# hanruihua/RDA-planner

Hardware: AMD Instinct MI355X
Metric: MPC steps/sec (ADMM early stop or iter_num cap: see residuals), T=20, N_obs=200 (higher is better)
Workload: dtype f64; 1 GPU; north-star: acker rectangle robot, T=20, N_obs=200 static seeded polygons, E=4, iter_num=4, iter_threshold=0.2, ro1=200; parallelism=single GPU

## Files before the change

include/rda_hip.h:

```cpp
#ifndef RDA_HIP_H
#define RDA_HIP_H
#include <stdint.h>
#ifdef __cplusplus
extern "C" {
#endif

#define RDA_EMAX 8
#define RDA_RMAX 8
#define RDA_TMAX 64

typedef struct rda_cfg {
    int32_t T;
    int32_t N;
    int32_t E;
    int32_t R;
    int32_t dynamics;
    int32_t accelerated;
    int32_t iter_num;
    int32_t robot_norm2;
    double dt, L;
    double max_speed[2];
    double acce_bound[2];
    double iter_threshold;
    double ws, wu;
// ... 214 lines not shown
                                     double *states_log , double *u_log , int32_t *index_log ,
                                     rda_info *info_log , int32_t *arrived_at ,
                                     int32_t *nbox_log , double *clearance_log ,
                                     double *peer_clearance_log , int see, double gate, int window);
int  rda_fleet_track_boxes(rda_fleet *f, const int32_t *n , const double *boxes , int cap, double gate, int window,
                           double *vel_out );
int  rda_fleet_box_tracks(rda_fleet *f, int cap, int32_t *n , double *centres, double *vel, int32_t *age);
int  rda_fleet_reset_tracks(rda_fleet *f, const int32_t *which , int count);
int  rda_set_scan_split(rda_handle *h, double tol);
int  rda_fleet_set_scan_split(rda_fleet *f, double tol);
int  rda_debug_fleet_world(rda_fleet *f, double *geom, int32_t *n_total, int32_t *we);
int  rda_fleet_enqueue_range(rda_fleet *f, int k0, int k1);
int  rda_fleet_sync(rda_fleet *f);

int  rda_get_state(rda_handle *h, double *lam, double *mu, double *z, double *xi, double *zeta,
                   double *dis, double *a_lam, double *b_lam);
int  rda_set_state(rda_handle *h, const double *lam, const double *mu, const double *z,
                   const double *xi, const double *zeta, const double *dis,
                   const double *a_lam, const double *b_lam);
#define RDA_SU_HISTORY_INTS 8
int  rda_get_su_history(rda_handle *h, int32_t *hist , double *lam_keep );
int  rda_set_su_history(rda_handle *h, const int32_t *hist , const double *lam_keep );
int  rda_get_su_history_n(rda_handle *h, int32_t *hist, int n_hist, double *lam_keep );
int  rda_set_su_history_n(rda_handle *h, const int32_t *hist, int n_hist, const double *lam_keep );
int  rda_lmz_history_doubles(rda_handle *h);
int  rda_get_lmz_history(rda_handle *h, double *points, int32_t *valid);
int  rda_set_lmz_history(rda_handle *h, const double *points, const int32_t *valid);
int  rda_debug_su_prof(rda_handle *h, long long *out16);
int  rda_debug_su_trace(rda_handle *h, long long *out, int cap, int *n_out);
int  rda_debug_su_land(rda_handle *h, int32_t *out4);
int  rda_debug_su_land_n(rda_handle *h, int32_t *out, int n);
int  rda_debug_flush_supports(rda_handle *h);
int  rda_debug_slot_src(rda_handle *h, int32_t *src , int32_t *used);
int  rda_debug_worklist(rda_handle *h, int *rows);
int  rda_debug_alloc_fail(int n);
int  rda_debug_alloc_stats(long long *live_allocs, long long *live_bytes);

int  rda_shard_config(rda_handle *h, int rank, int world);
int  rda_shard_chunk_doubles(rda_handle *h);
int  rda_shard_get_chunk(rda_handle *h, double *host_chunk);
int  rda_shard_set_chunks(rda_handle *h, const double *host_all);
int  rda_shard_unique_id(rda_handle *h, void *out128);
int  rda_shard_comm_init(rda_handle *h, const void *uid128);
int  rda_shard_comm_count(rda_handle *h);
int  rda_admm_begin(rda_handle *h, const double *nom_s, const double *nom_u, const double *ref_s, double ref_speed);
int  rda_admm_su(rda_handle *h, int it, int *stopped);
int  rda_admm_lammuz(rda_handle *h);
int  rda_admm_finish(rda_handle *h, double *out_u, double *out_s, rda_info *info);

int  rda_lammuz_batch(int B, int E, int R, const double *A, const double *b, const int32_t *cone,
                      const double *p, const double *phi, const double *G, const double *h,
                      const double *xi, const double *zeta, const double *dbar, double ro2, double delta,
                      int accelerated, double *lam, double *mu, double *z, double *cmh);

int  rda_su_solve(const rda_cfg *cfg, const double *nom_s, const double *nom_u, const double *ref_s,
                  double ref_speed, const double *a, const double *cc, const double *g,
                  const double *d0, double *s, double *u, double *d, int32_t *ipm_iters);
int  rda_su_solve_opts(const rda_cfg *cfg, const rda_opts *opts, const double *nom_s, const double *nom_u, const double *ref_s,
                       double ref_speed, const double *a, const double *cc, const double *g,
                       const double *d0, double *s, double *u, double *d, int32_t *ipm_iters);

#ifdef __cplusplus
}
#endif
#endif
```

rda_planner_amd/_capi.py:

```python
import ctypes as C
import numpy as np

c_double_p = C.POINTER(C.c_double)
c_int_p = C.POINTER(C.c_int)


class Cfg(C.Structure):
    _fields_ = [("T", C.c_int), ("N", C.c_int), ("E", C.c_int), ("R", C.c_int),
                ("dynamics", C.c_int), ("accelerated", C.c_int), ("iter_num", C.c_int),
                ("robot_norm2", C.c_int),
                ("dt", C.c_double), ("L", C.c_double),
                ("max_speed", C.c_double * 2), ("acce_bound", C.c_double * 2),
                ("iter_threshold", C.c_double), ("ws", C.c_double), ("wu", C.c_double),
                ("slack_gain", C.c_double), ("max_sd", C.c_double), ("min_sd", C.c_double),
                ("ro1", C.c_double), ("ro2", C.c_double),
                ("delta", C.c_double), ("eps_u", C.c_double)]


class Opts(C.Structure):
    _fields_ = [("lmz_mode", C.c_int), ("tie_centre", C.c_int), ("lmz_mu", C.c_double), ("su_tol", C.c_double * 3), ("su_tol_early", C.c_double * 3), ("su_hard_warm", C.c_double * 2),
                ("lmz_warm", C.c_int), ("lmz_rows", C.c_int), ("lmz_dense_from", C.c_int), ("lmz_split", C.c_int),
                ("lmz_ip_rows", C.c_int), ("lmz_ip_warm", C.c_int), ("su_pre", C.c_int), ("su_light", C.c_int),
                ("su_warm_first", C.c_int), ("su_warm_cap", C.c_int), ("su_easy_max", C.c_int), ("su_easy_nopred", C.c_int),
                ("su_cold_from", C.c_int), ("su_cold_probe", C.c_int), ("zero_copy", C.c_int), ("early_finish", C.c_int),
# ... 77 lines not shown
    "fleet_rollout_peers_plan": "i hiDDIdiiDDDDINIDDDI",
    "fleet_rollout_last_plan":  "i hD",
    "fleet_peer_clearance": "i hDD",
    "fleet_upload_worlds":  "i hIiIIDD",
    "fleet_raycast":        "i hIDDDDDD",
    "fleet_rollout_lidar":  "i hiDDIdiiDIDDDDdiIiDDINIID",
    "fleet_raycast_peers":  "i hIDDDDDD",
    "fleet_rollout_lidar_peers": "i hiDDIdiiDIDDDDdiIiDDINIIDD",
    "fleet_upload_scans_tracked": "i hIDDDDDdiIIdi",
    "fleet_rollout_lidar_tracked": "i hiDDIdiiDIDDDDdiIiDDINIIDDidi",
    "fleet_track_boxes":    "i hIDidiD",
    "fleet_box_tracks":     "i hiIDDI",
    "fleet_reset_tracks":   "i hIi",
    "set_scan_split":       "i hd",
    "fleet_set_scan_split": "i hd",
    "debug_fleet_world":    "i hDII",
    "fleet_enqueue_range":  "i hii",
    "fleet_sync":           "i h",
    "get_state":            "i hDDDDDDDD",
    "set_state":            "i hDDDDDDDD",
    "get_su_history":       "i hID",
    "set_su_history":       "i hID",
    "get_su_history_n":     "i hIiD",
    "set_su_history_n":     "i hIiD",
    "lmz_history_doubles":  "i h",
    "get_lmz_history":      "i hDI",
    "set_lmz_history":      "i hDI",
    "debug_su_prof":        "i hQ",
    "debug_su_trace":       "i hQiI",
    "debug_su_land":        "i hI",
    "debug_su_land_n":      "i hIi",
    "debug_flush_supports": "i h",
    "debug_slot_src":       "i hII",
    "debug_worklist":       "i hI",
    "debug_alloc_fail":     "i i",
    "debug_alloc_stats":    "i QQ",
    "shard_config":         "i hii",
    "shard_chunk_doubles":  "i h",
    "shard_get_chunk":      "i hD",
    "shard_set_chunks":     "i hD",
    "shard_unique_id":      "i hh",
    "shard_comm_init":      "i hh",
    "shard_comm_count":     "i h",
    "admm_begin":           "i hDDDd",
    "admm_su":              "i hiI",
    "admm_lammuz":          "i h",
    "admm_finish":          "i hDDN",
    "lammuz_batch":         "i iiiDDIDDDDDDDddiDDDD",
    "su_solve":             "i CDDDdDDDDDDDI",
    "su_solve_opts":        "i CODDDdDDDDDDDI",
    "debug_lmz_clk":        "i hhi",
    "debug_lmz_stats":      "i hh",
}
PROFILING_ONLY = frozenset(("debug_lmz_clk", "debug_lmz_stats"))


def signature(proto, codes=CODES):
    ret, _, params = proto.partition(" ")
    return codes[ret], [codes[c] for c in params]


def declare(lib, prefix, table, codes=CODES):
    for name, proto in table.items():
        fn = getattr(lib, f"{prefix}_{name}", None)
        if fn is not None:
            fn.restype, fn.argtypes = signature(proto, codes)
# ... 87 lines not shown
```

rda_planner_amd/csrc/rda_hip.hip:

```cpp
#include <hip/hip_runtime.h>
#include <cfloat>
#include <climits>
#include <cstdio>
#include <cstdlib>
#include <cstring>
#include <vector>
#include <chrono>
#include <memory>
#include <dlfcn.h>
#include "../../include/rda_hip.h"
#include "host_buf.h"
#include "lammuz_device.h"
#include "lammuz_cp_device.h"
#include "lammuz_ip_device.h"
#include "su_device.h"
#include "scene_device.h"
#include "lidar_device.h"
#include "track_device.h"
#include "rollout_device.h"

#define HIPCHK(x) do { hipError_t e_ = (x); if (e_ != hipSuccess) { \
    fprintf(stderr, "librda_hip: %s failed: %s (%s:%d)\n", #x, hipGetErrorString(e_), __FILE__, __LINE__); return RDA_ERR_HIP; } } while (0)

struct Ctrl {
// ... 263 lines not shown
    if (blind_opportunity && cl.blind_ok >= 0) a.land_blind = 1;
    if (!hard && a.warm_mu0 > 0 && d.su_cold_from > 0 && cl.su_last > d.su_cold_from && cl.su_last < 99 && cl.su_probe % d.su_cold_probe != d.su_cold_probe - 1) a.warm_mu0 = 0;
#ifdef SU_TRACE
    a.t_entry = t_entry_; t_mark_[3] = clock64();
    for (int k = 0; k < 4; ++k) a.t_mark[k] = t_mark_[k];
#endif
    su::solve<TT>(a, smem_su, pre, true, res, ref_wait);
    if (tid == 0) {
        const int su_last = res.status == 0 ? res.iters : 99;
        d.ctrl->iters = it + 1;
        if (res.status != 0) d.ctrl->su_status = cl.su_status | (1 << it);
        d.ctrl->ipm_iters = cl.ipm_iters + res.iters;
        d.ctrl->su_last = su_last;
        d.ctrl->su_hardlike = res.rd0 > su::HARD_RD0;
        d.ctrl->su_probe = (d.su_cold_from > 0 && su_last > d.su_cold_from && su_last < 99) ? cl.su_probe + 1 : 0;
        d.ctrl->pose_ok = 0;
        if (a.land) {
            const bool easy1 = res.status == 0 && res.iters == 0 && res.rounds_all == 1;
            d.ctrl->land_easy = easy1 ? (cl.land_easy < 8 ? cl.land_easy + 1 : 8) : 0;
            if (res.land_rho > 0) d.ctrl->land_rho_prev = res.land_rho;
            if (blind_opportunity) d.ctrl->blind_ok = res.blind == 1 ? (cl.blind_ok < 4 ? cl.blind_ok + 1 : 4) : (res.blind == 2 ? -6 : (cl.blind_ok < 0 ? cl.blind_ok + 1 : cl.blind_ok));
        }
        if (a.land && res.status == 0) {
            int lh = cl.land_hard;
            if (res.land_rounds >= 3) lh = 4; else if (lh > 0) lh -= 1;
            d.ctrl->land_hard = lh;
        }
        if (lf_eligible && d.su_land_first == 2) {
            int cr = cl.spec_credit;
            if (res.spec == 1) cr = cr + 3 > 6 ? 6 : cr + 3; else if (res.spec == 2) cr -= 2; else if (cr < 0) cr += 1;
            d.ctrl->spec_credit = cr;
        }
    }
}

template <int TT> __global__ __launch_bounds__(su::NT) void k_su(Dev d, int it, const double *in_s, const double *in_u, Fin fin)
{
    warm_kernargs<sizeof(Dev) + 2 * sizeof(void *) + sizeof(int) + sizeof(Fin)>();
    su_body<TT>(d, it, in_s, in_u, d.ref, d.ref_speed, nullptr, 0, &fin);
}

__device__ __forceinline__ void finish_body(const Dev &d, const Fin &f)
{
    if (d.ctrl->finished) return;
    if (!d.ctrl->stop && d.ctrl->resi_iter != d.ctrl->iters) { ResPre none; double rd, rp; reduce_residuals(d, threadIdx.x, d.ctrl->iters, none, false, nullptr, rd, rp); }
    __syncthreads();
    publish_result(d, f);
}

__global__ __launch_bounds__(su::NT) void k_finish(Dev d, Fin f) { finish_body(d, f); }

__device__ __forceinline__ void begin_body(const Dev &d)
{
    if (threadIdx.x == 0) {
        d.ctrl->stop = 0; d.ctrl->iters = 0; d.ctrl->su_status = 0; d.ctrl->ipm_iters = 0; d.ctrl->lmz_fail = 0;
        d.ctrl->resi_dual = 0; d.ctrl->resi_pri = 0; d.ctrl->finished = 0; d.ctrl->wl_count = 0; d.ctrl->wlc_count = 0; d.ctrl->resi_iter = 0;
    }
}

__global__ void k_begin(Dev d) { begin_body(d); }

__device__ __forceinline__ void prepare_body(const Dev &d, lmz::WaveLDS *wl)
{
    const int lane = threadIdx.x & 63, wv = threadIdx.x >> 6, E = d.c.E;
    const int w = blockIdx.x * 4 + wv;
    if (w >= d.c.N * d.nt) return;
// ... 196 lines not shown
constexpr int LMZ_CLK_WORDS = 32;
__device__ int *g_lmz_faillog = nullptr;
#endif
template <int MODE = 0, bool CW = false> __device__ __forceinline__ void lammuz_body_rows(const Dev &d, const int block, const int nblocks, const int it, const Fin &fin)
{
#pragma clang fp contract(on)
    constexpr int WPB = GS / 4;
    constexpr bool LANES = CW;
    __shared__ lmz::WaveLDS wl[GS];
    __shared__ lmz::RobotLDS rb;
    __shared__ double rowv[MODE == 0 ? GS : 1][6];
    const int T = d.c.T, E = d.c.E, R = d.c.R;
#ifdef RDA_LMZ_CLK
    long long clk_prev = clock64(); const long long clk_in = clk_prev; bool clk_enum = false; const unsigned long long clk_wall_in = (unsigned long long)wall_clock64();
    unsigned long long *const clk_slot = g_lmz_clk ? g_lmz_clk + LMZ_CLK_WORDS * (size_t)(block * (GS / 4) + (threadIdx.x >> 6)) : nullptr;
    long long clk_sub = clk_prev;
#define LMZ_CLK(k) do { if (MODE == 0) { const long long now_ = clock64(); if (clk_slot && (threadIdx.x & 63) == 0) clk_slot[k] += (unsigned long long)(now_ - clk_prev); clk_prev = now_; clk_sub = now_; } } while (0)
#define LMZ_SUB(k) do { if (MODE == 0) { const long long now_ = clock64(); if (clk_slot && (threadIdx.x & 63) == 0) clk_slot[16 + (k)] += (unsigned long long)(now_ - clk_sub); clk_sub = now_; } } while (0)
#else
#define LMZ_CLK(k) do { } while (0)
#define LMZ_SUB(k) do { } while (0)
#endif
    int tb = 0, jb = 0;
    if (MODE != 2) { block_of(d, block, tb, jb); if (tb < 0) return; }
    const int lane = threadIdx.x & 63, wv = threadIdx.x >> 6, row = lane >> 4, gl = lane & 15;
    struct Early { double px, py, cs, sn, xi0, xi1, zeta, dbar, prev, vtx[4], A, b, G, h, zold, rv; int cone, src, hpar, hint, npv, nlv; unsigned char lamc[3], muc; } ey;
    if (MODE == 0) {
        const int nl0 = jb * GS + wv * 4 + row, nl = nl0 < d.Nlive ? nl0 : 0, n = d.rank * d.Nloc + nl;
        ey.src = (d.slot_src && n < d.src_used) ? d.slot_src[n] : -1;
        ey.hpar = d.ctrl->hint_par & 1;
        static_assert(64 * WPB >= 56, "one element of the robot tables per thread");
        if (LANES) { ey.muc = d.muc[(int)threadIdx.x < 40 ? threadIdx.x : 0]; ey.rv = (&d.rv[0][0])[(int)threadIdx.x < 56 ? threadIdx.x : 0]; }
    }
    if (LANES) {
        int stop = d.ctrl->stop;
        asm volatile("" : "+v"(ey.hpar), "+v"(stop));
        ey.hpar = __builtin_amdgcn_readfirstlane(ey.hpar);
        if (__builtin_amdgcn_readfirstlane(stop)) return;
    } else
    if (d.ctrl->stop) return;
    if (MODE == 2 && block * WPB >= d.ctrl->wl_count + (d.ctrl->wlc_count + 3) / 4) return;
    LMZ_CLK(0);
    if (MODE == 0) {
        const int t = tb, nl0 = jb * GS + wv * 4 + row, nl = nl0 < d.Nlive ? nl0 : 0, n = d.rank * d.Nloc + nl;
        const double *ps = d.pose + 4 * t;
        const size_t o = drow(d, n, t + 1), zi = drow(d, n, t), oc = (size_t)n * d.nt + (d.nt > 1 ? t + 1 : 0);
        ey.px = ps[0]; ey.py = ps[1]; ey.cs = ps[2]; ey.sn = ps[3];
        ey.xi0 = d.xi[2 * o]; ey.xi1 = d.xi[2 * o + 1]; ey.zeta = d.zeta[zi]; ey.dbar = d.dis[t]; ey.cone = d.cone[n];
        ey.zold = d.z[zi];
        ey.prev = *(gl < E ? &d.lam[o * E + gl] : (gl < E + R ? &d.mu[o * R + gl - E] : &d.lam[o * E]));
        {
            const size_t ao = ((size_t)n * d.nt + (d.nt > 1 ? t + 1 : 0)) * E;
            ey.A = d.A[ao * 2 + (gl < 2 * E ? gl : 0)]; ey.b = d.b[ao + (gl < E ? gl : 0)];
            ey.G = d.G[(int)threadIdx.x < 2 * R ? threadIdx.x : 0]; ey.h = d.h[(int)threadIdx.x < R ? threadIdx.x : 0];
        }
#pragma unroll
        for (int k = 0; k < 3; ++k) ey.lamc[k] = gl + 16 * k < d.oc_ls ? d.oc_lamc[oc * d.oc_ls + gl + 16 * k] : (unsigned char)0;
#pragma unroll
        for (int k = 0; k < 4; ++k) ey.vtx[k] = gl + 16 * k < d.oc_vs ? d.oc_vtx[oc * d.oc_vs + gl + 16 * k] : 0.0;
        ey.npv = d.oc_cnt[2 * oc]; ey.nlv = d.oc_cnt[2 * oc + 1];
        {
            const int key = (ey.src >= 0 && ey.src < d.src_cap) ? d.c.N + ey.src : n, tr = (it == 0 && t + 1 < T) ? t + 1 : t;
            ey.hint = d.hint[(size_t)(ey.hpar ^ 1) * d.hint_len + (size_t)tr * d.hint_stride + key];
        }
    }
    LMZ_SUB(0);
    if (MODE == 0) {
        if ((int)threadIdx.x < 2 * R) rb.G[threadIdx.x >> 1][threadIdx.x & 1] = ey.G;
        if ((int)threadIdx.x < R) rb.h[threadIdx.x] = ey.h;
    } else {
        for (int i = threadIdx.x; i < 2 * R; i += 64 * WPB) rb.G[i >> 1][i & 1] = d.G[i];
        for (int i = threadIdx.x; i < R; i += 64 * WPB) rb.h[i] = d.h[i];
    }
    if (LANES) {
        if ((int)threadIdx.x < 40) rb.muc[threadIdx.x] = ey.muc;
        if ((int)threadIdx.x < 56) (&rb.rv[0][0])[threadIdx.x] = ey.rv;
    } else {
        for (int i = threadIdx.x; i < 40; i += 64 * WPB) rb.muc[i] = d.muc[i];
        for (int i = threadIdx.x; i < 56; i += 64 * WPB) (&rb.rv[0][0])[i] = (&d.rv[0][0])[i];
    }
    if (threadIdx.x == 0) { rb.nmv = d.nmv; rb.nrv = d.nrv; }
    LMZ_SUB(1);
    const int cntP = MODE == 2 ? d.ctrl->wl_count : 1, cntC = MODE == 2 ? d.ctrl->wlc_count : 0;
    const int cnt = cntP + (cntC + 3) / 4;
    for (int base = MODE == 2 ? block * WPB : 0; base < cnt; base += MODE == 2 ? nblocks * WPB : 1) {
    if (MODE == 2) __syncthreads();
    const bool entry = MODE == 2 && base + wv < cnt;
    int t, nl;
    bool live2 = false;
    if (MODE == 2) {
        const int sl = entry ? base + wv : base;
        int widx;
        if (sl < cntP) { widx = sl; live2 = entry && row == 0; }
// ... 973 lines not shown
extern "C" int rda_debug_su_trace(rda_handle *H, long long *out, int cap, int *n_out)
{
    if (!H || !out || !n_out || cap < 1) return RDA_ERR_ARG;
#if defined(SU_TRACE)
    if (!H->d.su_prof) return RDA_ERR_UNSUPPORTED;
    HIPCHK(hipStreamSynchronize(H->stream));
    std::vector<long long> buf(2 * 4 * su::TRACE_CAP);
    HIPCHK(hipMemcpy(buf.data(), H->d.su_prof + 16, buf.size() * sizeof(long long), hipMemcpyDeviceToHost));
    const int n = cap < su::TRACE_CAP ? cap : su::TRACE_CAP;
    for (int w = 0; w < 4; ++w)
        for (int e = 0; e < n; ++e) { out[(w * cap + e) * 2] = buf[(w * su::TRACE_CAP + e) * 2]; out[(w * cap + e) * 2 + 1] = buf[(w * su::TRACE_CAP + e) * 2 + 1]; }
    *n_out = n;
    return RDA_OK;
#else
    (void)H;
    return RDA_ERR_UNSUPPORTED;
#endif
}

extern "C" int rda_debug_flush_supports(rda_handle *H)
{
    if (!H) return RDA_ERR_ARG;
    HIPCHK(hipMemsetAsync(H->d.hint, 0xff, 2 * (size_t)H->d.hint_len * sizeof(int), H->stream));
    HIPCHK(hipStreamSynchronize(H->stream));
    return RDA_OK;
}
extern "C" int rda_debug_slot_src(rda_handle *H, int32_t *src, int32_t *used)
{
    if (!H || !src || !used) return RDA_ERR_ARG;
    HIPCHK(hipStreamSynchronize(H->stream));
    if (H->tick.scene_on_s2) HIPCHK(hipStreamSynchronize(H->stream2));
    *used = H->d.slot_src ? H->d.src_used : 0;
    if (*used > 0) HIPCHK(hipMemcpy(src, H->d.slot_src, (size_t)*used * sizeof(int), hipMemcpyDeviceToHost));
    return RDA_OK;
}
extern "C" int rda_debug_worklist(rda_handle *H, int *rows)
{
    if (!H || !rows) return RDA_ERR_ARG;
    HIPCHK(hipStreamSynchronize(H->stream));
    HIPCHK(hipMemcpy(rows, &H->d.ctrl->wl_count, sizeof(int), hipMemcpyDeviceToHost));
    return RDA_OK;
}
extern "C" int rda_debug_alloc_fail(int n) { hbuf::refuse_in = n; return RDA_OK; }
extern "C" int rda_debug_alloc_stats(long long *live_allocs, long long *live_bytes)
{
    if (live_allocs) *live_allocs = hbuf::live_allocs;
    if (live_bytes) *live_bytes = hbuf::live_bytes;
    return RDA_OK;
}

static int obstacles_stage(rda_handle *H, int n_obs, const double *A, const double *b, const int32_t *cone, int per_t, bool sync)
{
    if (!H) return RDA_ERR_ARG;
    Dev &d = H->d;
    const size_t T = d.c.T, N = d.c.N, E = d.c.E;
    if (n_obs <= 0) { d.obstacle_num = 0; return RDA_OK; }
    if (!A || !b || !cone) return RDA_ERR_ARG;
    if (H->opts.duals_follow) return RDA_ERR_UNSUPPORTED;
    d.sc_bad = nullptr;
    H->sc.n = 0;
    const size_t nt = per_t ? T + 1 : 1;
    for (size_t n = 0; n < N; ++n) {
        size_t src = n < (size_t)n_obs ? n : (size_t)n_obs - 1;
        memcpy(&H->stage.A[n * nt * E * 2], &A[src * nt * E * 2], nt * E * 2 * sizeof(double));
        memcpy(&H->stage.b[n * nt * E], &b[src * nt * E], nt * E * sizeof(double));
        H->stage.cone[n] = cone[src];
// ... 2698 lines not shown
```

rda_planner_amd/csrc/su_device.h:

```cpp
#pragma once
#include <hip/hip_runtime.h>
#include <math.h>

#ifndef SIGMA_FLOOR
#define SIGMA_FLOOR 1e-3
#endif
#define SU_CENTRE_GAMMA 1e-5
#define SU_CENTRE_FROM 25
#define SU_SMOOTH_K 0.1
#define SU_COLD_CAP 50
#define SU_SAFE_SIGMA 0.3
#define SU_SAFE_SIGMA_END 0.05
#define SU_SAFE_TAU 0.9
#define SU_SAFE_GAMMA 1e-2
#pragma clang fp contract(on)

namespace su {

constexpr int NT = 256;
constexpr double HARD_RD0 = 1e-2, HARD_DMU = 1.0;
constexpr int NC = 10;
constexpr int LAND_STATS = 20;
constexpr int TRACE_CAP = 1024;
#ifdef SU_TRACE
// ... 222 lines not shown
    __syncthreads();
    double r = slots[0];
    for (int w = 1; w < NT / 64; ++w) r = is_max ? (slots[w] > r ? slots[w] : r) : r + slots[w];
    return r;
}

__device__ __forceinline__ void con_T(const double *x, int t, double &y3, double &y4, double &y5, double &y6, double &y7)
{
    double r0 = t >= 1 ? x[6] - x[7] : 0.0, r1 = t >= 1 ? x[8] - x[9] : 0.0;
    y5 = x[0] - x[1] + r0; y6 = x[2] - x[3] + r1; y7 = x[4] - x[5]; y3 = -r0; y4 = -r1;
}

__device__ __forceinline__ double Fel(const double *Ft_t, int i, int q) { return Ft_t[6 * q + i]; }

template <int TT> __device__ __forceinline__ bool pair_map(const int T, const int j, int &t, int &k)
{
    const int tid = threadIdx.x, lane = tid & 63, wave = tid >> 6;
    if (TT > 0 && TT <= 32) {
        const int half = lane >> 5, tl = lane & 31;
        k = wave == 0 ? half : (wave == 1 ? 3 + half : 2);
        const bool ok = j == 0 && tl < T && (wave < 2 || (wave == 2 && half == 0));
        t = ok ? tl : 0; if (!ok) k = 0;
        return ok;
    }
    const int pi = tid + j * NT;
    const bool ok = pi < 5 * T;
    t = ok ? pi / 5 : 0; k = ok ? pi % 5 : 0;
    return ok;
}

#ifndef SU_LAND_FALLBACK
#define SU_LAND_FALLBACK 1e-3
#endif
struct Result { int status = 1, iters = 0; double rd0 = 0; int spec = 0; int land_rounds = 0; int rounds_all = 0; int blind = 0; double land_rho = 0; };
struct Pre {
    double vref = 0;
    double u0 = 0, u1 = 0, d = 0, cp = 0, sp = 0;
    double lkp[2] = {0, 0}, lkm[2] = {0, 0};
    double q0[8], q1[8], q2[8]; unsigned long long mk[8];
    double sv = 0, rv = 0;
    double p0a = 0, p0b = 0;
};
template <int TT> __device__ __forceinline__ void prefetch(const Args &a, Pre &p)
{
    const Cfg &c = a.c;
    const int T = TT > 0 ? TT : c.T, tid = threadIdx.x;
    p.vref = *a.ref_speed;
    p.d = c.max_sd;
    if (tid < 128 && (tid & 63) < T) {
        const int t = tid & 63;
        p.u0 = a.in_u[t]; p.u1 = a.in_u[T + t]; if (a.d_in) p.d = a.d_in[t];
        if (a.pose_lin) { p.cp = a.pose[4 * t + 2]; p.sp = a.pose[4 * t + 3]; }
    }
    if (a.lam_keep)
        for (int j = 0; j < 2; ++j) {
            int t, kk;
            if (pair_map<TT>(T, j, t, kk)) {
                const int ts = a.warm_shift ? (t + 1 < T ? t + 1 : T - 1) : t;
                p.lkp[j] = a.lam_keep[ts * NC + 2 * kk]; p.lkm[j] = a.lam_keep[ts * NC + 2 * kk + 1];
            }
        }
    const int nch = NT / T, rt = tid / nch, rc_ = tid % nch;
#pragma unroll
    for (int k = 0; k < 8; ++k) { p.q0[k] = 0; p.q1[k] = 0; p.q2[k] = 0; p.mk[k] = 0; }
    if (a.bsum != nullptr && rt < T) {
        const int J = a.J, KB = (J + nch - 1) / nch;
        const double *bs = a.bsum + (size_t)rt * J * NBS;
// ... 106 lines not shown
#pragma unroll
            for (int q = 0; q < 3; ++q) F[6 * q + r] = Am[3 * r + q];
#pragma unroll
            for (int q = 0; q < 2; ++q) F[6 * (5 + q) + r] = Bm[2 * r + q];
        }
        F[6 * 5 + 3] = 1.0; F[6 * 6 + 4] = 1.0;
    }
    if (wave == 1 && lane < T) {
        const int t = lane;
        const double clipm = warm ? a.warm_clip : 0.01;
        const double lim0 = (1.0 - clipm) * c.umax0, lim1 = (1.0 - clipm) * c.umax1;
        const double v0 = pf_u0, v1 = pf_u1;
        L.u[t] = v0 > lim0 ? lim0 : (v0 < -lim0 ? -lim0 : v0);
        L.u[T + t] = v1 > lim1 ? lim1 : (v1 < -lim1 ? -lim1 : v1);
        const double lo = c.min_sd + clipm * (c.max_sd - c.min_sd), hi = c.max_sd - clipm * (c.max_sd - c.min_sd);
        const double dv = pf_d;
        L.d[t] = dv > hi ? hi : (dv < lo ? lo : dv);
    }
    __syncthreads();
    MS(11); TR(131);
    auto clip_controls = [&](const double clipm) {
        if (tid < T) {
            int t = tid;
            double lim0 = (1.0 - clipm) * c.umax0, lim1 = (1.0 - clipm) * c.umax1;
            double v0 = pf_u0, v1 = pf_u1;
            L.u[t] = v0 > lim0 ? lim0 : (v0 < -lim0 ? -lim0 : v0);
            L.u[T + t] = v1 > lim1 ? lim1 : (v1 < -lim1 ? -lim1 : v1);
            double lo = c.min_sd + clipm * (c.max_sd - c.min_sd), hi = c.max_sd - clipm * (c.max_sd - c.min_sd);
            double dv = pf_d;
            L.d[t] = dv > hi ? hi : (dv < lo ? lo : dv);
        }
        __syncthreads();
    };
    auto rollout = [&](const int wv = 0) {
        if (wave == wv) {
            double *inc = L.dy;
            for (int t = lane; t < T; t += 64) {
                const double *B = &L.Bk[6 * t], *C = &L.Ck[3 * t];
                const double u0 = L.u[t], u1 = L.u[T + t];
                inc[3 * t + 2] = (B[4] * u0 + B[5] * u1) + C[2];
                inc[3 * t] = (B[0] * u0 + B[1] * u1) + C[0];
                inc[3 * t + 1] = (B[2] * u0 + B[3] * u1) + C[1];
            }
            wsync();
            auto prefix = [&](double v) {
                v += dpp_f64<0x111>(v); v += dpp_f64<0x112>(v); v += dpp_f64<0x114>(v); v += dpp_f64<0x118>(v);
                v += dpp_f64<0x142, 0xA>(v); v += dpp_f64<0x143, 0xC>(v);
                return v;
            };
            {
                const double ph0 = L.s[2 * (T + 1)];
                const double v = prefix(lane < T ? inc[3 * lane + 2] : 0.0);
                if (lane < T) L.s[2 * (T + 1) + lane + 1] = ph0 + v;
            }
            wsync();
            {
                const double x0 = L.s[0], y0 = L.s[T + 1];
                double ix = 0, iy = 0;
                if (lane < T) {
                    const double ph = L.s[2 * (T + 1) + lane];
                    ix = inc[3 * lane] + L.Ak[9 * lane + 2] * ph; iy = inc[3 * lane + 1] + L.Ak[9 * lane + 5] * ph;
                }
                const double px = prefix(ix), py = prefix(iy);
                if (lane < T) { L.s[lane + 1] = x0 + px; L.s[(T + 1) + lane + 1] = y0 + py; }
            }
        }
    };
    rollout(3);
    MS(13); TR(133);
    constexpr int NPR = TT > 0 ? (5 * TT + NT - 1) / NT : 2;
    int  p_t[NPR], p_k[NPR]; bool p_ok[NPR], p_on[NPR];
    double p_ep[NPR], p_em[NPR];
    double Pwp[NPR], Pwm[NPR], Plp[NPR], Plm[NPR];
    double Prpp[NPR], Prpm[NPR], Prcp[NPR], Prcm[NPR];
    double Piwp[NPR], Piwm[NPR], Pilp[NPR], Pilm[NPR];
    double Pdwp[NPR], Pdwm[NPR], Pdlp[NPR], Pdlm[NPR];
#pragma unroll
    for (int j = 0; j < NPR; ++j) {
        p_ok[j] = pair_map(j, p_t[j], p_k[j]);
        p_on[j] = p_ok[j] && (p_k[j] < 3 || p_t[j] >= 1);
        p_ep[j] = con_rhs(c, 2 * p_k[j]); p_em[j] = con_rhs(c, 2 * p_k[j] + 1);
        Pwp[j] = Pwm[j] = 1.0; Plp[j] = Plm[j] = 0.0; Prpp[j] = Prpm[j] = Prcp[j] = Prcm[j] = 0.0;
        Piwp[j] = Piwm[j] = 1.0; Pilp[j] = Pilm[j] = 0.0; Pdwp[j] = Pdwm[j] = Pdlp[j] = Pdlm[j] = 0.0;
    }
    auto frcp = [](double x) {
        double r = __builtin_amdgcn_rcp(x);
        r = __builtin_fma(r, __builtin_fma(-x, r, 1.0), r);
        return __builtin_fma(r, __builtin_fma(-x, r, 1.0), r);
    };
    auto pair_val = [&](int t, int k) {
        if (k == 2) return L.d[t];
        const double *uu = (k == 1 || k == 4) ? &L.u[T] : &L.u[0];
        const double v = uu[t];
        return k < 3 ? v : v - (t ? uu[t - 1] : 0.0);
    };
    auto pair_step = [&](int t, int k) {
        const double *y = &L.dy[8 * t], *v = &L.vv[8 * t + 3];
        if (k == 2) {
// ... 505 lines not shown
            x = sum8(x);
            if (q == 0) XS_x0[j] = x;
        }
    };
    auto interface_solve = [&](double &xm, double &pi) {
        const int j = lane < 5 ? lane : 0;
        double si[5], xx[5], pmv[5], pj[5];
#pragma unroll
        for (int k2 = 0; k2 < 5; ++k2) { si[k2] = XS_SI[5 * j + k2]; xx[k2] = XS_X[5 * j + k2]; pmv[k2] = XS_pm[k2]; pj[k2] = Px[8 * j + k2]; }
        double rr = XS_x0[j], w = XS_pm[j];
#pragma unroll
        for (int k2 = 0; k2 < 5; ++k2) rr += xx[k2] * pmv[k2];
        double v = 0.0;
        asm volatile("s_nop 1\n\t"
                     "v_fmac_f64_dpp %0, %1, %2 row_newbcast:0 row_mask:0xf bank_mask:0xf\n\t"
                     "v_fmac_f64_dpp %0, %1, %3 row_newbcast:1 row_mask:0xf bank_mask:0xf\n\t"
                     "v_fmac_f64_dpp %0, %1, %4 row_newbcast:2 row_mask:0xf bank_mask:0xf\n\t"
                     "v_fmac_f64_dpp %0, %1, %5 row_newbcast:3 row_mask:0xf bank_mask:0xf\n\t"
                     "v_fmac_f64_dpp %0, %1, %6 row_newbcast:4 row_mask:0xf bank_mask:0xf"
                     : "+v"(v) : "v"(rr), "v"(si[0]), "v"(si[1]), "v"(si[2]), "v"(si[3]), "v"(si[4]));
        xm = v;
        asm volatile("s_nop 1\n\t"
                     "v_fmac_f64_dpp %0, %1, %2 row_newbcast:0 row_mask:0xf bank_mask:0xf\n\t"
                     "v_fmac_f64_dpp %0, %1, %3 row_newbcast:1 row_mask:0xf bank_mask:0xf\n\t"
                     "v_fmac_f64_dpp %0, %1, %4 row_newbcast:2 row_mask:0xf bank_mask:0xf\n\t"
                     "v_fmac_f64_dpp %0, %1, %5 row_newbcast:3 row_mask:0xf bank_mask:0xf\n\t"
                     "v_fmac_f64_dpp %0, %1, %6 row_newbcast:4 row_mask:0xf bank_mask:0xf"
                     : "+v"(w) : "v"(xm), "v"(pj[0]), "v"(pj[1]), "v"(pj[2]), "v"(pj[3]), "v"(pj[4]));
        pi = w;
    };

    int status = 1, it = 0, used = 0;
    bool have_acc = false; double acc_merit = 0.0;
    if (tid == 0) { *flag_meas = 0; *flag_stop = 0; *flag_fail = 0; *flag_unit = 0; *flag_unit2 = 0; }
    bool ref_pending = a.ref_flag != nullptr;
    MS(9); TR(101);
    for (int attempt = a.first_attempt ? 1 : (warm ? -1 : 0); attempt < 2 && status != 0; ++attempt) {
    const bool safe = attempt == 1;
    double al_prev = 0.0;
    int land = 0, land_rounds = 0, land_its = 0;
    int land_level = a.land_level0;
    double land_rho = 0.0;
    bool expect_conv = attempt < 0 && a.land != 0 && a.land_first != 0;
    int spec_dec = 0;
    bool blind = false;
    bool spec = false, spec_tried = false;
    auto land_refuse = [&](const bool last) {
        __syncthreads();
        for (int i = tid; i < 2 * T; i += NT) L.u[i] = L.sav[i];
        for (int i = tid; i < T; i += NT) L.d[i] = L.sav[2 * T + i];
#pragma unroll
        for (int j = 0; j < NPR; ++j) { Pwp[j] = Swp[j]; Pwm[j] = Swm[j]; Plp[j] = Slp[j]; Plm[j] = Slm[j]; }
        __syncthreads();
        rollout();
        __syncthreads();
        LSTAT(1, 1);
        land = 0; expect_conv = false;
        if (blind) { blind = false; res.blind = 2; }
        if (spec) { spec = false; spec_tried = true; res.spec = 2; } else land_level = last ? 99 : land_level + 1;
        pair_rows();
        __syncthreads();
    };
    if (attempt == 1 || (attempt == 0 && warm)) {
        __syncthreads();
        clip_controls(0.01);
        rollout();
        __syncthreads();
// ... 561 lines not shown
                al_prev = al;
                if (recentre) {
                    const double floor_ = (safe ? SU_SAFE_GAMMA : SU_CENTRE_GAMMA) * m_;
#pragma unroll
                    for (int j = 0; j < NPR; ++j)
                        if (p_on[j]) {
                            if (Plp[j] * Pwp[j] < floor_) Plp[j] = floor_ / Pwp[j];
                            if (Plm[j] * Pwm[j] < floor_) Plm[j] = floor_ / Pwm[j];
                        }
                    pair_rows();
                    __syncthreads();
                }
                const double prd = (1 - al) * rdn, prp = (1 - al) * rpn;
                expect_conv = c.light_check && ((prd <= t_rd * sc && prp <= t_rp && m_ <= t_mu * sc) ||
                                                (prd <= 100 * t_rd * sc && prp <= t_rp && m_ <= 0.1 * t_mu * sc));
            }
            mark(8);
        }
    }
    used += it - land_its > 0 ? it - land_its : 0;
    LSTAT(3, land_its);
    }
    __syncthreads();
    if ((status != 0 || a.accept == 2) && have_acc) {
        for (int i = tid; i < 2 * T; i += NT) L.u[i] = L.acc[i];
        for (int i = tid; i < T; i += NT) L.d[i] = L.acc[2 * T + i];
#pragma unroll
        for (int j = 0; j < NPR; ++j)
            if (p_ok[j]) { const int o = 3 * T + 10 * p_t[j] + 2 * p_k[j]; Plp[j] = L.acc[o]; Plm[j] = L.acc[o + 1]; }
        status = 0;
        __syncthreads();
    }
    TR(102);
    rollout();
    __syncthreads();
    mark(15); TR(103);
    if (status == 0 && a.lam_keep) {
#pragma unroll
        for (int j = 0; j < NPR; ++j)
            if (p_ok[j]) { const int o = p_t[j] * NC + 2 * p_k[j]; a.lam_keep[o] = p_on[j] ? Plp[j] : 0.0; a.lam_keep[o + 1] = p_on[j] ? Plm[j] : 0.0; }
    }
    if (status == 0) {
        for (int i = tid; i < 3 * (T + 1); i += NT) a.out_s[i] = L.s[i];
        for (int i = tid; i < 2 * T; i += NT) a.out_u[i] = L.u[i];
        for (int i = tid; i < T; i += NT) a.out_d[i] = L.d[i];
    } else if (a.out_s != a.in_s) {
        for (int i = tid; i < 3 * (T + 1); i += NT) a.out_s[i] = a.in_s[i];
        for (int i = tid; i < 2 * T; i += NT) a.out_u[i] = a.in_u[i];
        if (a.d_in) for (int i = tid; i < T; i += NT) a.out_d[i] = a.d_in[i];
    }
    if (a.pose_out && tid < T) {
        const bool okk = status == 0;
        const double px = okk ? L.s[tid + 1] : a.in_s[tid + 1], py = okk ? L.s[(T + 1) + tid + 1] : a.in_s[(T + 1) + tid + 1];
        const double ph = okk ? L.s[2 * (T + 1) + tid] : a.in_s[2 * (T + 1) + tid];
        double sp, cp; sincos(ph, &sp, &cp);
        a.pose_out[4 * tid] = px; a.pose_out[4 * tid + 1] = py; a.pose_out[4 * tid + 2] = cp; a.pose_out[4 * tid + 3] = sp;
    }
    if (tid == 0) { *a.status = status; *a.ipm_iters = used; }
    res.status = status; res.iters = used;
    mark(10); TR(104);
    if (prof_on && tid == 0) for (int k = 0; k < 16; ++k) a.prof[k] += pacc[k];
    return true;
}
#undef RW
#undef LSTAT
#undef R5
#undef MS
#undef MF
#undef LDS_DRAIN
#undef TR

}

#pragma clang fp contract(fast)
```

Baseline: 4289 steps/s.

## Overlap SU tail rollout with pose sincos and output stores across waves

Splits the end of the SU solve across waves. Wave 0 runs the final rollout and publishes an LDS flag once the heading is ready. Wave 1 spins on that flag and computes the pose sincos while the x/y prefix sums are still running, and the remaining waves write the u/d outputs and status at the same time. The LMZ kernel also moves its stop-flag check in the latency mode until after the initial loads, so that load latency is overlapped with the stop test. The intent is to shorten the serial tail of each SU call, at the cost of an intra-block spin-wait and more complex wave-specialised code; a debug pose readback and trace hooks are added as well.

```diff
diff --git a/include/rda_hip.h b/include/rda_hip.h
--- a/include/rda_hip.h
+++ b/include/rda_hip.h
@@ -270,6 +270,7 @@
 int  rda_debug_su_land_n(rda_handle *h, int32_t *out, int n);
 int  rda_debug_flush_supports(rda_handle *h);
 int  rda_debug_slot_src(rda_handle *h, int32_t *src , int32_t *used);
+int  rda_debug_pose(rda_handle *h, double *pose , double *s );
 int  rda_debug_worklist(rda_handle *h, int *rows);
 int  rda_debug_alloc_fail(int n);
 int  rda_debug_alloc_stats(long long *live_allocs, long long *live_bytes);
diff --git a/rda_planner_amd/_capi.py b/rda_planner_amd/_capi.py
--- a/rda_planner_amd/_capi.py
+++ b/rda_planner_amd/_capi.py
@@ -133,6 +133,7 @@
     "debug_su_land_n":      "i hIi",
     "debug_flush_supports": "i h",
     "debug_slot_src":       "i hII",
+    "debug_pose":           "i hDD",
     "debug_worklist":       "i hI",
     "debug_alloc_fail":     "i i",
     "debug_alloc_stats":    "i QQ",
diff --git a/rda_planner_amd/csrc/rda_hip.hip b/rda_planner_amd/csrc/rda_hip.hip
--- a/rda_planner_amd/csrc/rda_hip.hip
+++ b/rda_planner_amd/csrc/rda_hip.hip
@@ -319,6 +319,9 @@
             d.ctrl->spec_credit = cr;
         }
     }
+#ifdef SU_TRACE
+    if (a.prof && (tid & 63) == 0 && res.trn < su::TRACE_CAP) { long long *q = a.prof + 16 + ((tid >> 6) * su::TRACE_CAP + res.trn) * 2; q[0] = 110; q[1] = clock64(); }
+#endif
 }
 
 template <int TT> __global__ __launch_bounds__(su::NT) void k_su(Dev d, int it, const double *in_s, const double *in_u, Fin fin)
@@ -581,15 +584,13 @@
         static_assert(64 * WPB >= 56, "one element of the robot tables per thread");
         if (LANES) { ey.muc = d.muc[(int)threadIdx.x < 40 ? threadIdx.x : 0]; ey.rv = (&d.rv[0][0])[(int)threadIdx.x < 56 ? threadIdx.x : 0]; }
     }
-    if (LANES) {
-        int stop = d.ctrl->stop;
-        asm volatile("" : "+v"(ey.hpar), "+v"(stop));
-        ey.hpar = __builtin_amdgcn_readfirstlane(ey.hpar);
-        if (__builtin_amdgcn_readfirstlane(stop)) return;
-    } else
-    if (d.ctrl->stop) return;
+    LMZ_SUB(14);
+    static_assert(!LANES || MODE == 0, "the latency form takes its stop test inside the mode-0 batch");
+    int stop = 0;
+    if (LANES) { stop = d.ctrl->stop; asm volatile("" ::: "memory"); }
+    else if (d.ctrl->stop) return;
     if (MODE == 2 && block * WPB >= d.ctrl->wl_count + (d.ctrl->wlc_count + 3) / 4) return;
-    LMZ_CLK(0);
+    if (!LANES) LMZ_CLK(0);
     if (MODE == 0) {
         const int t = tb, nl0 = jb * GS + wv * 4 + row, nl = nl0 < d.Nlive ? nl0 : 0, n = d.rank * d.Nloc + nl;
         const double *ps = d.pose + 4 * t;
@@ -608,6 +609,14 @@
 #pragma unroll
         for (int k = 0; k < 4; ++k) ey.vtx[k] = gl + 16 * k < d.oc_vs ? d.oc_vtx[oc * d.oc_vs + gl + 16 * k] : 0.0;
         ey.npv = d.oc_cnt[2 * oc]; ey.nlv = d.oc_cnt[2 * oc + 1];
+        if (LANES) {
+            asm volatile("" ::: "memory");
+            LMZ_SUB(15);
+            asm volatile("" : "+v"(ey.hpar), "+v"(stop));
+            ey.hpar = __builtin_amdgcn_readfirstlane(ey.hpar);
+            if (__builtin_amdgcn_readfirstlane(stop)) return;
+            LMZ_CLK(0);
+        }
         {
             const int key = (ey.src >= 0 && ey.src < d.src_cap) ? d.c.N + ey.src : n, tr = (it == 0 && t + 1 < T) ? t + 1 : t;
             ey.hint = d.hint[(size_t)(ey.hpar ^ 1) * d.hint_len + (size_t)tr * d.hint_stride + key];
@@ -1647,6 +1656,15 @@
     if (H->tick.scene_on_s2) HIPCHK(hipStreamSynchronize(H->stream2));
     *used = H->d.slot_src ? H->d.src_used : 0;
     if (*used > 0) HIPCHK(hipMemcpy(src, H->d.slot_src, (size_t)*used * sizeof(int), hipMemcpyDeviceToHost));
+    return RDA_OK;
+}
+extern "C" int rda_debug_pose(rda_handle *H, double *pose, double *s)
+{
+    if (!H || !pose || !s) return RDA_ERR_ARG;
+    HIPCHK(hipStreamSynchronize(H->stream));
+    const size_t T = H->d.c.T;
+    HIPCHK(hipMemcpy(pose, H->d.pose, 4 * T * sizeof(double), hipMemcpyDeviceToHost));
+    HIPCHK(hipMemcpy(s, H->d.s, 3 * (T + 1) * sizeof(double), hipMemcpyDeviceToHost));
     return RDA_OK;
 }
 extern "C" int rda_debug_worklist(rda_handle *H, int *rows)
diff --git a/rda_planner_amd/csrc/su_device.h b/rda_planner_amd/csrc/su_device.h
--- a/rda_planner_amd/csrc/su_device.h
+++ b/rda_planner_amd/csrc/su_device.h
@@ -278,7 +278,11 @@
 #ifndef SU_LAND_FALLBACK
 #define SU_LAND_FALLBACK 1e-3
 #endif
-struct Result { int status = 1, iters = 0; double rd0 = 0; int spec = 0; int land_rounds = 0; int rounds_all = 0; int blind = 0; double land_rho = 0; };
+struct Result { int status = 1, iters = 0; double rd0 = 0; int spec = 0; int land_rounds = 0; int rounds_all = 0; int blind = 0; double land_rho = 0;
+#ifdef SU_TRACE
+    int trn = 0;
+#endif
+};
 struct Pre {
     double vref = 0;
     double u0 = 0, u1 = 0, d = 0, cp = 0, sp = 0;
@@ -451,7 +455,8 @@
         }
         __syncthreads();
     };
-    auto rollout = [&](const int wv = 0) {
+    unsigned long long *const flag_head = reinterpret_cast<unsigned long long *>(L.pv + 6);
+    auto rollout = [&](const int wv = 0, const bool tail = false) {
         if (wave == wv) {
             double *inc = L.dy;
             for (int t = lane; t < T; t += 64) {
@@ -473,6 +478,7 @@
                 if (lane < T) L.s[2 * (T + 1) + lane + 1] = ph0 + v;
             }
             wsync();
+            if (tail) { if (lane == 0) __atomic_store_n(flag_head, 1ull, __ATOMIC_RELEASE); TR(105); }
             {
                 const double x0 = L.s[0], y0 = L.s[T + 1];
                 double ix = 0, iy = 0;
@@ -483,6 +489,7 @@
                 const double px = prefix(ix), py = prefix(iy);
                 if (lane < T) { L.s[lane + 1] = x0 + px; L.s[(T + 1) + lane + 1] = y0 + py; }
             }
+            if (tail) { TR(106); }
         }
     };
     rollout(3);
@@ -1054,7 +1061,7 @@
 
     int status = 1, it = 0, used = 0;
     bool have_acc = false; double acc_merit = 0.0;
-    if (tid == 0) { *flag_meas = 0; *flag_stop = 0; *flag_fail = 0; *flag_unit = 0; *flag_unit2 = 0; }
+    if (tid == 0) { *flag_meas = 0; *flag_stop = 0; *flag_fail = 0; *flag_unit = 0; *flag_unit2 = 0; *flag_head = 0; }
     bool ref_pending = a.ref_flag != nullptr;
     MS(9); TR(101);
     for (int attempt = a.first_attempt ? 1 : (warm ? -1 : 0); attempt < 2 && status != 0; ++attempt) {
@@ -1682,33 +1689,58 @@
         __syncthreads();
     }
     TR(102);
-    rollout();
+    const bool okk = status == 0;
+    auto keep_store = [&]() {
+        if (okk && a.lam_keep) {
+#pragma unroll
+            for (int j = 0; j < NPR; ++j)
+                if (p_ok[j]) { const int o = p_t[j] * NC + 2 * p_k[j]; a.lam_keep[o] = p_on[j] ? Plp[j] : 0.0; a.lam_keep[o + 1] = p_on[j] ? Plm[j] : 0.0; }
+        }
+    };
+    const bool copy_nom = !okk && a.out_s != a.in_s;
+    double pose_x = 0, pose_y = 0, pose_c = 0, pose_s = 0;
+    if (wave == 0) rollout(0, true);
+    else if (wave == 1) {
+        if (a.pose_out) {
+            double ph = 0;
+            if (okk) {
+                while (__atomic_load_n(flag_head, __ATOMIC_ACQUIRE) != 1ull) __builtin_amdgcn_s_sleep(1);
+                TR(109);
+                if (lane < T) ph = L.s[2 * (T + 1) + lane];
+            } else if (lane < T) { pose_x = a.in_s[lane + 1]; pose_y = a.in_s[(T + 1) + lane + 1]; ph = a.in_s[2 * (T + 1) + lane]; }
+            if (lane < T) sincos(ph, &pose_s, &pose_c);
+            TR(108);
+        }
+        keep_store();
+    } else {
+        keep_store();
+        const int NW = NT - 2 * 64;
+        if (okk) {
+            for (int i = tid - 2 * 64; i < 2 * T; i += NW) a.out_u[i] = L.u[i];
+            for (int i = tid - 2 * 64; i < T; i += NW) a.out_d[i] = L.d[i];
+        } else if (copy_nom) {
+            for (int i = tid - 2 * 64; i < 3 * (T + 1); i += NW) a.out_s[i] = a.in_s[i];
+            for (int i = tid - 2 * 64; i < 2 * T; i += NW) a.out_u[i] = a.in_u[i];
+            if (a.d_in) for (int i = tid - 2 * 64; i < T; i += NW) a.out_d[i] = a.d_in[i];
+        }
+        if (tid == 2 * 64) { *a.status = status; *a.ipm_iters = used; }
+        TR(107);
+    }
     __syncthreads();
     mark(15); TR(103);
-    if (status == 0 && a.lam_keep) {
-#pragma unroll
-        for (int j = 0; j < NPR; ++j)
-            if (p_ok[j]) { const int o = p_t[j] * NC + 2 * p_k[j]; a.lam_keep[o] = p_on[j] ? Plp[j] : 0.0; a.lam_keep[o + 1] = p_on[j] ? Plm[j] : 0.0; }
-    }
-    if (status == 0) {
-        for (int i = tid; i < 3 * (T + 1); i += NT) a.out_s[i] = L.s[i];
-        for (int i = tid; i < 2 * T; i += NT) a.out_u[i] = L.u[i];
-        for (int i = tid; i < T; i += NT) a.out_d[i] = L.d[i];
-    } else if (a.out_s != a.in_s) {
-        for (int i = tid; i < 3 * (T + 1); i += NT) a.out_s[i] = a.in_s[i];
-        for (int i = tid; i < 2 * T; i += NT) a.out_u[i] = a.in_u[i];
-        if (a.d_in) for (int i = tid; i < T; i += NT) a.out_d[i] = a.d_in[i];
-    }
-    if (a.pose_out && tid < T) {
-        const bool okk = status == 0;
-        const double px = okk ? L.s[tid + 1] : a.in_s[tid + 1], py = okk ? L.s[(T + 1) + tid + 1] : a.in_s[(T + 1) + tid + 1];
-        const double ph = okk ? L.s[2 * (T + 1) + tid] : a.in_s[2 * (T + 1) + tid];
-        double sp, cp; sincos(ph, &sp, &cp);
-        a.pose_out[4 * tid] = px; a.pose_out[4 * tid + 1] = py; a.pose_out[4 * tid + 2] = cp; a.pose_out[4 * tid + 3] = sp;
-    }
-    if (tid == 0) { *a.status = status; *a.ipm_iters = used; }
+    if (wave == 0) keep_store();
+    else if (wave == 1) {
+        if (a.pose_out && lane < T) {
+            if (okk) { pose_x = L.s[lane + 1]; pose_y = L.s[(T + 1) + lane + 1]; }
+            a.pose_out[4 * lane] = pose_x; a.pose_out[4 * lane + 1] = pose_y; a.pose_out[4 * lane + 2] = pose_c; a.pose_out[4 * lane + 3] = pose_s;
+        }
+    } else if (okk)
+        for (int i = tid - 2 * 64; i < 3 * (T + 1); i += NT - 2 * 64) a.out_s[i] = L.s[i];
     res.status = status; res.iters = used;
     mark(10); TR(104);
+#ifdef SU_TRACE
+    res.trn = trn;
+#endif
     if (prof_on && tid == 0) for (int k = 0; k < 16; ++k) a.prof[k] += pacc[k];
     return true;
 }
```

Result: no change. 4311 steps/s, median of 3 (+0.5%).
